# narendasan/irl-maxent

Hardware: AMD Instinct MI355X
Metric: IRL gradient steps/sec (VI + SVF sweep), NxN grid batch B (higher is better)
Workload: dtype f64

## Files before the change

irl-maxent_amd/csrc/cluster.h:

```cpp
#pragma once

#include <hip/hip_runtime.h>
#include <stdint.h>

#include "common.h"

namespace irlmx {

constexpr int kCT = 1024;
constexpr int kSptMax = 6;
constexpr int kPairThreads = 512;
constexpr int kSptMaxPair = 12;
constexpr int kSptMaxQuadFwd = 12;
constexpr int kSptMaxQuadBwd = 16;
constexpr int kSptMaxQuadBwdCW = 20;
constexpr int kTMax = 16;
constexpr int kSoloBwdT = 256;
constexpr int kRescaleEvery = 32;
constexpr size_t kMaxLdsBytes = 160 * 1024;
constexpr int kSumSlots = kRescaleEvery < 8 ? 8 : kRescaleEvery + 1;
static_assert(kSumSlots > kRescaleEvery, "summary slots must outlast the rescale period");
constexpr int kSumRows = kSumSlots + 2;
constexpr int kXccRow = kSumSlots, kFullRow = kSumSlots + 1;
constexpr size_t kClusterStaticLds = 128;
constexpr int kModeFwd = 0;
constexpr int kModeBwd = 1;

struct ClusterArgs {
  int W, H, S, A;
  int R, G, C, T;
  int b0;
  int nb;
  int btot;
  int emax;
  int tab_shared;
  const double* wgt;
  const double* row_val;
  const double* vin;
  const uint8_t* term;
  const int32_t* bad;
  const unsigned long long* growth;
  double eps;
  long long max_iter;
  long long n_sweeps;
  int rescale;
  unsigned long long* gran;
  unsigned long long* sgran;
  int xcd_group;
  unsigned salt;
  int* err;
  int n_resident;
  unsigned long long gather_ticks;
  int test_drop;
  int eager_summary;
  unsigned long long* stamps;
  double* out;
  int64_t* iters;
  int32_t* status;
};

struct ClusterPlan {
  int R, G, C, T, per_launch, spt, emax;
  size_t lds;
  int pair;
  int nt;
};

typedef unsigned int u32x4 __attribute__((ext_vector_type(4)));
constexpr int kPollSleep = 1;
constexpr int kGatherPerThread = 4;

#ifndef IRLMX_GRAN_PAR_PAD
#define IRLMX_GRAN_PAR_PAD -1
#endif
#ifndef IRLMX_GRAN_INST_PAD
#define IRLMX_GRAN_INST_PAD -1
#endif
__host__ __device__ inline size_t gran_par_pad(int W) { return IRLMX_GRAN_PAR_PAD >= 0 ? IRLMX_GRAN_PAR_PAD : (W == 128 ? 24 : 0); }
__host__ __device__ inline size_t gran_inst_pad(int W) { return IRLMX_GRAN_INST_PAD >= 0 ? IRLMX_GRAN_INST_PAD : (W == 128 ? 40 : 0); }
__host__ __device__ inline size_t gran_par_len(int W, int H) { return (size_t)H * W + gran_par_pad(W); }
__host__ __device__ inline size_t gran_inst_len(int W, int H) { return 2 * gran_par_len(W, H) + gran_inst_pad(W); }

struct Gran {
  __amdgpu_buffer_rsrc_t r;
#if IRLMX_DEVICE_CHECKS
  unsigned bytes;
#endif
};
__device__ inline Gran gran_rsrc(const void* base, unsigned bytes) {
  Gran g;
  g.r = __builtin_amdgcn_make_buffer_rsrc(const_cast<void*>(base), 0, (int)bytes, 0x00020000);
#if IRLMX_DEVICE_CHECKS
  g.bytes = bytes;
#endif
  return g;
}
#if IRLMX_DEVICE_CHECKS
__device__ inline bool gran_in(const Gran& g, unsigned off) { return g.bytes >= 16u && off <= g.bytes - 16u; }
#endif
__device__ inline unsigned long long dbits(double v) { return (unsigned long long)__double_as_longlong(v); }
__device__ inline void gran_store(const Gran& g, unsigned off, unsigned long long v, unsigned tag, bool plain) {
  if (!IRLMX_DCHECK(gran_in(g, off), kCheckGranule)) return;
  const u32x4 x = {(unsigned)v, tag, (unsigned)(v >> 32), tag};
  if (plain) __builtin_amdgcn_raw_buffer_store_b128(x, g.r, (int)off, 0, 0);
  else __builtin_amdgcn_raw_buffer_store_b128(x, g.r, (int)off, 0, 16 );
}
constexpr unsigned long long kGatherTicks = 2000000000ull;
// ... 100 lines not shown
```

irl-maxent_amd/csrc/cluster.hip:

```cpp

#include <hip/hip_runtime.h>

#include <algorithm>
#include <atomic>
#include <cmath>
#include <cstdio>
#include <cstdlib>
#include <type_traits>

#include "cluster.h"
#include "common.h"

namespace irlmx {

template <int CTRL>
__device__ inline double dpp_shift_f64(double x) {
  const long long b = __double_as_longlong(x);
  const int lo = __builtin_amdgcn_update_dpp(0, (int)(b & 0xffffffffLL), CTRL, 0xF, 0xF, true);
  const int hi = __builtin_amdgcn_update_dpp(0, (int)(b >> 32), CTRL, 0xF, 0xF, true);
  return __longlong_as_double(((long long)hi << 32) | (long long)(unsigned)lo);
}

template <int MODE, int SPT, int WT, int LAY, int NT>
__global__ void __launch_bounds__(NT) cluster_kernel(ClusterArgs a) {
  constexpr bool PAIR = LAY >= 1, COLS = LAY >= 2;
  constexpr bool CW = LAY == 4;
  constexpr int CPL = LAY >= 3 ? 4 : 2;
  static_assert(LAY != 1 || (SPT % 2 == 0 && (WT == 64 || WT == 128)), "pair rows: even SPT, width 64/128");
  static_assert(LAY != 2 || (SPT % 2 == 0 && (WT == 64 || WT == 128)), "column pairs: even SPT, width 64/128");
  static_assert(LAY != 3 || (SPT % 4 == 0 && (WT == 128 || WT == 256)), "column quads: SPT % 4, width 128/256");
  static_assert(LAY != 4 || (MODE == kModeBwd && SPT % 4 == 0 && WT == 256), "compact weights: backward, width 256");
  constexpr int RW = COLS ? SPT / CPL : 1;
  constexpr int HW = COLS ? WT / CPL : 1;
  constexpr int NB = COLS ? NT / HW : 1;
  constexpr int QW = CPL / 2;
  constexpr bool kProof = MODE == kModeFwd && COLS;
  constexpr int kProofRow = RW / 2;
  constexpr bool kLdsSides = COLS && CPL == 2 && MODE == kModeFwd;
  extern __shared__ __attribute__((aligned(16))) unsigned char smem[];
  const int W = WT ? WT : a.W;
  const int H = a.H, S = a.S;
  int lin = blockIdx.x;
  if (a.xcd_group) {
    const int g = blockIdx.x % 8, k = blockIdx.x / 8;
    const int il = g + 8 * (k / a.C);
    if (il >= a.nb) return;
    lin = il * a.C + k % a.C;
  }
  const int tile = lin % a.C;
  const int inst = a.b0 + lin / a.C;
  const int tid = threadIdx.x;
  {
    __shared__ int resident;
    if (tid == 0) resident = coresident(a.err + 1, a.n_resident) ? 1 : 0;
    __syncthreads();
    if (!resident) {
      if (tid == 0) atomicOr(a.err, kErrNotResident);
      return;
    }
  }
  if (lin == a.test_drop) return;
  const int r0 = tile * a.R, r1 = min(H, r0 + a.R);
  const int e0 = max(0, r0 - a.G), e1 = min(H, r1 + a.G);
  const int E = (e1 - e0) * W;
  if (!IRLMX_DCHECK(0 <= e0 && e0 <= r0 && r0 < r1 && r1 <= e1 && e1 <= H && E <= a.emax && E <= SPT * NT,
                    kCheckTile))
    return;
  const int own0 = (r0 - e0) * W, own1 = (r1 - e0) * W;
  const int pubA1 = min(own1, own0 + a.G * W), pubB0 = max(pubA1, own1 - a.G * W);
  const int base = e0 * W;
  const int pad = PAIR ? W : W + 1;
  const int blen = a.emax + 2 * pad;
  const int cp = COLS ? tid % HW : 0, bb = COLS ? tid / HW : 0;
  auto slot_state = [&](int j) {
    if (COLS) return (bb * RW + j / CPL) * W + CPL * cp + j % CPL;
    return PAIR ? 2 * (tid + (j >> 1) * NT) + (j & 1) : tid + j * NT;
  };
  double* bufA = (double*)smem;
  double* bufB = bufA + (COLS ? 0 : blen);
  double* snap = bufB + blen;
  constexpr int kBndLen = COLS ? 2 * (NB + 2) * 2 * HW * QW : 0;
  double2* bnd = CW ? (double2*)bufA : (double2*)(snap + (MODE == kModeFwd ? a.emax : 0));
  unsigned char* tail = CW ? (unsigned char*)bufA + max((size_t)blen * sizeof(double), (size_t)kBndLen * sizeof(double2))
                           : (unsigned char*)(bnd + kBndLen);
  double2* wmid = (double2*)tail;
  double2* zrow = wmid + (CW ? NB * RW * HW : 0);
  unsigned long long* red = (unsigned long long*)(zrow + (CW ? HW * QW : 0));
  int* lflag = (int*)(red + 3);

  const size_t iS = (size_t)inst * S;
  if (MODE == kModeFwd && a.bad[inst]) {
    for (int l = own0 + tid; l < own1; l += NT) a.out[iS + base + l] = __longlong_as_double(0x7ff8000000000000LL);
    if (tile == 0 && tid == 0) { a.iters[inst] = 1; a.status[inst] = IRLMX_NONFINITE; }
    return;
  }

  double w[CW ? 1 : SPT][kStencilK];
  double wc[CW ? SPT : 1][3];
  double edge_w[CW ? 2 * RW : 1];
  double c0[MODE == kModeFwd ? SPT : 1];
  const size_t wbase = iS * kStencilK;
#pragma unroll
  for (int j = 0; j < SPT; ++j) {
    const int l = slot_state(j);
    if (MODE == kModeFwd) c0[MODE == kModeFwd ? j : 0] = 0.0;
    if constexpr (CW) {
#pragma unroll
      for (int k = 0; k < 3; ++k) wc[j][k] = 0.0;
      if (l < E) {
        const int s = base + l;
        const int x = s % W;
        wc[j][0] = a.wgt[wbase + (size_t)(x + 1 < W ? 1 : 2) * S + s];
        wc[j][1] = a.wgt[wbase + (size_t)3 * S + s];
        wc[j][2] = a.wgt[wbase + (size_t)4 * S + s];
      }
#pragma unroll
      for (int k = 0; k < 3; ++k) asm volatile("" : "+v"(wc[j][k]));
    } else {
#pragma unroll
      for (int k = 0; k < kStencilK; ++k) w[j][k] = 0.0;
      if (l < E) {
        const int s = base + l;
        if (MODE == kModeFwd) c0[MODE == kModeFwd ? j : 0] = a.vin[iS + s];
#pragma unroll
        for (int k = 0; k < kStencilK; ++k) w[j][k] = a.wgt[wbase + (size_t)k * S + s];
      }
#pragma unroll
      for (int k = 0; k < kStencilK; ++k) asm volatile("" : "+v"(w[j][k]));
      if (MODE == kModeFwd) asm volatile("" : "+v"(c0[MODE == kModeFwd ? j : 0]));
    }
  }
  if constexpr (CW) {
#pragma unroll
    for (int r = 0; r < RW; ++r) {
      edge_w[2 * r] = 0.0;
      edge_w[2 * r + 1] = 0.0;
      const int l0 = slot_state(r * CPL), l3 = slot_state(r * CPL + CPL - 1);
      const int y = e0 + l0 / W;
      const bool brow = l0 < E && (y == 0 || y == H - 1);
      if ((cp == 0 || brow) && l0 < E) edge_w[2 * r] = a.wgt[wbase + base + l0];
      if ((cp == HW - 1 || brow) && l3 < E) edge_w[2 * r + 1] = a.wgt[wbase + base + l3];
      asm volatile("" : "+v"(edge_w[2 * r]));
      asm volatile("" : "+v"(edge_w[2 * r + 1]));
    }
  }
  auto finish = [&](int j, double acc) { return MODE == kModeFwd ? c0[MODE == kModeFwd ? j : 0] + acc : acc; };
  bool wave_p0 = true;
  if constexpr (MODE == kModeFwd) {
    bool mine = false;
#pragma unroll
    for (int j = 0; j < SPT; ++j) mine |= !(c0[MODE == kModeFwd ? j : 0] == 0.0);
    wave_p0 = __builtin_amdgcn_readfirstlane(__builtin_amdgcn_ballot_w64(mine) != 0ull ? 1 : 0) != 0;
  }
  for (int i = tid; i < (COLS ? 1 : 2) * blen; i += NT) bufA[i] = 0.0;
  for (int i = tid; i < kBndLen; i += NT) bnd[i] = make_double2(0.0, 0.0);
  if constexpr (CW) {
    static_assert(!CW || CPL == 4, "compact weights: column quads");
    for (int i = tid; i < HW * QW; i += NT) zrow[i] = make_double2(0.0, 0.0);
#pragma unroll
    for (int r = 0; r < RW; ++r) {
      const int l1 = slot_state(r * CPL + 1);
      const int y = e0 + l1 / W;
      const bool brow = l1 < E && (y == 0 || y == H - 1);
      wmid[(bb * RW + r) * HW + cp] = brow ? make_double2(a.wgt[wbase + base + l1], a.wgt[wbase + base + l1 + 1])
                                           : make_double2(0.0, 0.0);
    }
  }
  __syncthreads();
  for (int l = tid; l < E; l += NT) {
    double v0 = 0.0;
    if (MODE == kModeBwd) v0 = a.term[iS + base + l] ? 1.0 : 0.0;
    bufA[pad + l] = v0;
    bufB[pad + l] = v0;
    if (MODE == kModeFwd) snap[l] = v0;
  }
  if (tid < 3) red[tid] = 0ull;
  if (tid == 0) lflag[0] = 0;
  double cv[PAIR ? SPT : 1];
#pragma unroll
  for (int j = 0; j < (PAIR ? SPT : 1); ++j) {
    const int l = slot_state(j);
    cv[j] = (PAIR && MODE == kModeBwd && l < E) ? (a.term[iS + base + l] ? 1.0 : 0.0) : 0.0;
  }
  auto reload = [&](const double* buf) {
    if (PAIR) {
#pragma unroll
      for (int j = 0; j < (PAIR ? SPT : 1); ++j) cv[j] = buf[pad + slot_state(j)];
    }
  };

  unsigned own_bits = 0, pub_bits = 0, ext_bits = 0;
#pragma unroll
  for (int j = 0; j < SPT; ++j) {
    const int l = slot_state(j);
    const bool own = l >= own0 && l < own1;
    own_bits |= (own ? 1u : 0u) << j;
    ext_bits |= (l < E ? 1u : 0u) << j;
    pub_bits |= (((l >= own0 && l < pubA1) || (l >= pubB0 && l < own1)) ? 1u : 0u) << j;
  }

  constexpr bool kUniformSlots = LAY == 1 ? WT == 128 : (COLS && HW == 64);
  auto slot_bits = [&](unsigned b) {
    if constexpr (kUniformSlots) {
      b = (unsigned)__builtin_amdgcn_readfirstlane((int)b);
      asm volatile("" : "+s"(b));
    } else {
      asm volatile("" : "+v"(b));
    }
    return b;
  };

  int T = a.T;
  int p_max = 1;
  if (MODE == kModeBwd) {
    const double g = bits_double(a.growth[inst]);
    const double d = bits_double(a.growth[a.btot + inst]);
    if (a.rescale && isfinite(g)) {
      int cap = 1 << 20;
      if (g > 1.0) cap = max(1, (int)floor(900.0 / log2(g)) - 1);
      if (d > 0.0 && d < 1.0) cap = min(cap, max(1, (int)floor(900.0 / -log2(d)) - 1));
      if (d < 0.0) cap = min(cap, kTMax);
      T = max(1, min(T, cap));
      p_max = d < 0.0 ? 1 : max(1, min(kRescaleEvery, cap / T));
    }
  }
  __syncthreads();

  const double eps = a.eps;
  auto sweep = [&](const double* __restrict__ din, double* __restrict__ dout, int i, unsigned& flags) {
    const unsigned ob = slot_bits(own_bits);
    double dmax = 0.0;
    auto account = [&](int j, double nv, double self) {
      if (MODE == kModeFwd && ((ob >> j) & 1u)) dmax = fmax(dmax, fabs(nv - self));
    };
    if constexpr (PAIR && !COLS) {
#pragma unroll
      for (int jp = 0; jp < SPT / 2; ++jp) {
        const int l = 2 * (tid + jp * NT);
        const double2 up = *reinterpret_cast<const double2*>(din + l);
        const double2 dn = *reinterpret_cast<const double2*>(din + 2 * W + l);
        const double va = cv[2 * jp], vb = cv[2 * jp + 1];
        const double lft = dpp_shift_f64<0x138>(vb);
        const double rgt = dpp_shift_f64<0x130>(va);
        const double* wa = w[CW ? 0 : 2 * jp];
        const double* wb = w[CW ? 0 : 2 * jp + 1];
        double acc = fma(wa[0], va, 0.0);
        acc = fma(wa[1], vb, acc);
        acc = fma(wa[2], lft, acc);
        acc = fma(wa[3], dn.x, acc);
        acc = fma(wa[4], up.x, acc);
        const double na = finish(2 * jp, acc);
        acc = fma(wb[0], vb, 0.0);
        acc = fma(wb[1], rgt, acc);
        acc = fma(wb[2], va, acc);
        acc = fma(wb[3], dn.y, acc);
        acc = fma(wb[4], up.y, acc);
        const double nb = finish(2 * jp + 1, acc);
        *reinterpret_cast<double2*>(dout + W + l) = make_double2(na, nb);
        account(2 * jp, na, va);
        account(2 * jp + 1, nb, vb);
        cv[2 * jp] = na;
        cv[2 * jp + 1] = nb;
      }
    } else {
#pragma unroll
      for (int j = 0; j < SPT; ++j) {
        const int l = tid + j * NT;
        const double* q = din + l + 1;
        const double self = q[W];
        double acc = fma(w[CW ? 0 : j][0], self, 0.0);
        acc = fma(w[CW ? 0 : j][1], q[W + 1], acc);
        acc = fma(w[CW ? 0 : j][2], q[W - 1], acc);
        acc = fma(w[CW ? 0 : j][3], q[2 * W], acc);
        acc = fma(w[CW ? 0 : j][4], q[0], acc);
        const double nv = finish(j, acc);
        dout[pad + l] = nv;
        account(j, nv, self);
      }
    }
    if (MODE == kModeFwd) flags |= ((dmax > eps) ? 1u : 0u) << i;
    __syncthreads();
  };

  double cw[COLS ? SPT : 1];
  auto bnd_at = [&](int par, int band, int e) { return bnd + ((((size_t)par * (NB + 2) + band) * 2 + e) * HW + cp) * QW; };
  auto cols_sweep = [&](const double (&src)[COLS ? SPT : 1], double (&dst)[COLS ? SPT : 1], int i,
                        unsigned& flags, auto p0tag, auto fulltag) {
    constexpr bool kP0 = decltype(p0tag)::value;
    constexpr bool kFull = decltype(fulltag)::value;
    if constexpr (COLS) {
      const unsigned ob = slot_bits(own_bits);
      double dmax = 0.0;
      double2 wm_pf[CW ? RW : 1];
      if constexpr (CW) {
#pragma unroll
        for (int r = 0; r < RW; ++r) wm_pf[r] = wmid[(bb * RW + r) * HW + cp];
      }
      auto account = [&](int j, double nv, double self) {
        if (!kFull && j / CPL != kProofRow) return;
        if constexpr (MODE == kModeFwd && kUniformSlots) {
          if ((ob >> j) & 1u) {
            asm volatile("");
            dmax = fmax(dmax, fabs(nv - self));
          }
        } else if (MODE == kModeFwd && ((ob >> j) & 1u)) {
          dmax = fmax(dmax, fabs(nv - self));
        }
      };
      {
        double2* t = bnd_at(i & 1, bb + 1, 0);
        double2* u = bnd_at(i & 1, bb + 1, 1);
#pragma unroll
        for (int q = 0; q < QW; ++q) {
          t[q] = make_double2(src[2 * q], src[2 * q + 1]);
          u[q] = make_double2(src[SPT - CPL + 2 * q], src[SPT - CPL + 2 * q + 1]);
        }
      }
      constexpr bool kBwdPairs12 = CPL == 2 && MODE == kModeBwd && SPT >= 12;
      constexpr bool kPinStores = CPL == 2 && MODE == kModeBwd && (SPT <= 8 || kBwdPairs12);
      if constexpr (kPinStores) __builtin_amdgcn_sched_barrier(0);
      if (MODE == kModeFwd && i == 0) {
        const unsigned xb = slot_bits(ext_bits);
#pragma unroll
        for (int jp = 0; jp < SPT / 2; ++jp)
          if ((xb >> (2 * jp)) & 1u)
            *reinterpret_cast<double2*>(snap + slot_state(2 * jp)) = make_double2(src[2 * jp], src[2 * jp + 1]);
      }
      double above[CPL], below[CPL];
      double side[2][2];
      constexpr bool kPin = CPL == 2 && !kBwdPairs12;
      auto edges_in = [&]() {
        if (kPin) __builtin_amdgcn_sched_barrier(0);
        __syncthreads();
        if (kPin) __builtin_amdgcn_sched_barrier(0);
        const double2* t = (CW && bb == 0) ? zrow + cp * QW : bnd_at(i & 1, bb, 1);
        const double2* u = (CW && bb == NB - 1) ? zrow + cp * QW : bnd_at(i & 1, bb + 2, 0);
#pragma unroll
        for (int q = 0; q < QW; ++q) {
          const double2 x = t[q];
// ... 26 lines not shown
          double acc[CPL];
          if constexpr (CW) {
            const double2 wm = wm_pf[jr];
            acc[0] = fma(edge_w[2 * jr], v[0], 0.0);
            acc[1] = fma(wm.x, v[1], 0.0);
            acc[2] = fma(wm.y, v[2], 0.0);
            acc[CPL - 1] = fma(edge_w[2 * jr + 1], v[CPL - 1], 0.0);
#pragma unroll
            for (int c = 0; c < CPL; ++c) acc[c] = fma(wc[jr * CPL + c][0], c + 1 < CPL ? v[c + 1 < CPL ? c + 1 : 0] : rgt, acc[c]);
#pragma unroll
            for (int c = 0; c < CPL; ++c) acc[c] = fma(wc[jr * CPL + c][0], c > 0 ? v[c > 0 ? c - 1 : 0] : lft, acc[c]);
#pragma unroll
            for (int c = 0; c < CPL; ++c) acc[c] = fma(wc[jr * CPL + c][1], dn[c], acc[c]);
#pragma unroll
            for (int c = 0; c < CPL; ++c) acc[c] = fma(wc[jr * CPL + c][2], up[c], acc[c]);
          } else {
#pragma unroll
            for (int c = 0; c < CPL; ++c) acc[c] = fma(w[CW ? 0 : jr * CPL + c][0], v[c], 0.0);
#pragma unroll
            for (int c = 0; c < CPL; ++c) acc[c] = fma(w[CW ? 0 : jr * CPL + c][1], c + 1 < CPL ? v[c + 1 < CPL ? c + 1 : 0] : rgt, acc[c]);
#pragma unroll
            for (int c = 0; c < CPL; ++c) acc[c] = fma(w[CW ? 0 : jr * CPL + c][2], c > 0 ? v[c > 0 ? c - 1 : 0] : lft, acc[c]);
#pragma unroll
            for (int c = 0; c < CPL; ++c) acc[c] = fma(w[CW ? 0 : jr * CPL + c][3], dn[c], acc[c]);
#pragma unroll
            for (int c = 0; c < CPL; ++c) acc[c] = fma(w[CW ? 0 : jr * CPL + c][4], up[c], acc[c]);
          }
#pragma unroll
          for (int c = 0; c < CPL; ++c) {
            dst[jr * CPL + c] = kP0 ? finish(jr * CPL + c, acc[c]) : acc[c];
            account(jr * CPL + c, dst[jr * CPL + c], v[c]);
          }
        }
      };
      constexpr int step = CPL == 2 ? 2 : 1;
      constexpr int n_int = RW >= 3 ? (RW - 2 + step - 1) / step : 0;
      constexpr int kPre = (CW || kBwdPairs12) ? n_int
                           : (CPL == 2 && MODE == kModeFwd && SPT <= 8) ? 0
                                                                       : (n_int + 1) / 2;
#pragma unroll
      for (int s = 0; s < n_int; ++s) {
        if (s == kPre) edges_in();
        const int jp = 1 + s * step;
        rows(jp, jp + step - 1 <= RW - 2 ? jp + step - 1 : jp);
      }
      if constexpr (kPre >= n_int) edges_in();
      if constexpr (RW >= 2) {
        if constexpr (CPL == 2) rows(RW - 1, 0);
        else { rows(RW - 1, RW - 1); rows(0, 0); }
      } else {
        rows(0, 0);
      }
      if (MODE == kModeFwd) flags |= ((dmax > eps) ? 1u : 0u) << i;
    }
  };

  const size_t gpl = gran_par_len(W, H);
  const Gran rg = gran_rsrc(a.gran + (size_t)inst * 2 * gran_inst_len(W, H), 32u * (unsigned)gpl);
  const unsigned rgw = (unsigned)W;
  const unsigned gbase = (unsigned)e0 * rgw;
  auto gidx = [&](int l) { return gbase + (unsigned)(l / W) * rgw + (unsigned)(l % W); };
  const Gran rs = gran_rsrc(a.sgran + (size_t)inst * 2 * kSumRows * a.H, 16u * kSumRows * (unsigned)a.H);
  const int ng0 = own0, ng = own0 + (E - own1);
  const unsigned salt = (a.salt & 0xFFFu) << 20;
  bool plain = false;
  {
    unsigned xcc;
    asm volatile("s_getreg_b32 %0, hwreg(HW_REG_XCC_ID)" : "=s"(xcc));
    xcc &= 0xFu;
    const unsigned htag = salt | 0xFFFFFu;
    if (tid == 0) gran_store(rs, ((unsigned)kXccRow * (unsigned)a.H + (unsigned)tile) * 16u, xcc, htag, false);
    bool ok = true;
    if (tid < kWave) {
      unsigned long long diff = 0ull;
      for (int t0 = 0; t0 < a.C; t0 += kWave) {
        unsigned long long v[1] = {xcc};
        unsigned off[1] = {((unsigned)kXccRow * (unsigned)a.H + (unsigned)(t0 + tid)) * 16u};
        ok &= gran_gather<1>(rs, rs, off, t0 + tid < a.C ? 1u : 0u, htag, v, a.gather_ticks);
        diff |= v[0] ^ xcc;
      }
      diff = wave_or_u64(diff);
      if (tid == 0) { red[2] = diff; lflag[1] = ok ? 0 : 1; }
    }
    __syncthreads();
    if (lflag[1]) { if (tid == 0) atomicOr(a.err, 1); return; }
    plain = a.xcd_group && red[2] == 0ull;
    __syncthreads();
  }

  double* cur = bufA;
  double* oth = bufB;
  long long done = 0;
  __shared__ unsigned long long st_acc[8], ts_l[1];
  const bool stamps = a.stamps != nullptr && tid == 0;
  if (stamps) {
    for (int k = 0; k < 8; ++k) st_acc[k] = 0ull;
    ts_l[0] = stamp_now();
  }
  unsigned long long& ts = ts_l[0];
  auto stamp = [&](int k) {
    if (stamps) { const unsigned long long t = stamp_now(); st_acc[k] += t - ts; ts = t; }
  };
  auto stamp_flush = [&]() {
    if (stamps) {
      for (int k = 0; k < 5; ++k) a.stamps[(size_t)lin * 8 + k] = st_acc[k];
      a.stamps[(size_t)lin * 8 + 5] = plain ? 1 : 0;
// ... 3 lines not shown
  };
  const long long total = MODE == kModeBwd ? a.n_sweeps : -1;
  int rescale_in = 1;
  auto run_sweeps = [&](int n, unsigned& fl) {
    if constexpr (COLS) {
      int i = 0;
      for (; i + 1 < n; i += 2) {
        cols_sweep(cv, cw, i, fl, std::true_type{}, std::true_type{});
        cols_sweep(cw, cv, i + 1, fl, std::true_type{}, std::true_type{});
      }
      if (i < n) {
        cols_sweep(cv, cw, i, fl, std::true_type{}, std::true_type{});
#pragma unroll
        for (int j = 0; j < (COLS ? SPT : 1); ++j) cv[j] = cw[j];
      }
    } else {
      for (int i = 0; i < n; ++i) {
        sweep(cur, oth, i, fl);
        double* t = cur; cur = oth; oth = t;
      }
    }
  };
  auto restore = [&]() {
    for (int l = tid; l < E; l += NT) cur[pad + l] = snap[l];
    __syncthreads();
    reload(cur);
  };
  auto block_sweeps = [&](unsigned& fl, const int n, auto fulltag) {
    if constexpr (COLS && MODE == kModeFwd) {
      auto go = [&](auto p0tag) {
        int i = 0;
        for (; i + 1 < n; i += 2) {
          cols_sweep(cv, cw, i, fl, p0tag, fulltag);
          cols_sweep(cw, cv, i + 1, fl, p0tag, fulltag);
        }
        if (i < n) {
          cols_sweep(cv, cw, i, fl, p0tag, fulltag);
#pragma unroll
          for (int j = 0; j < (COLS ? SPT : 1); ++j) cv[j] = cw[j];
        }
      };
      if (MODE == kModeFwd && ((decltype(fulltag)::value && kProof) || wave_p0)) go(std::true_type{});
      else go(std::false_type{});
    }
  };
  for (int m = 0;; ++m) {
    int Tm = T;
    if (MODE == kModeBwd) Tm = (int)min<long long>((long long)T, total - done);
    unsigned flags = 0;
    const bool resc = MODE == kModeBwd && a.rescale && (rescale_in <= 1 || done + Tm >= total);
    double mxd = 0.0;
    if constexpr (COLS) {
      if constexpr (MODE == kModeBwd) {
        int i = 0;
        for (; i + 1 < Tm; i += 2) {
          cols_sweep(cv, cw, i, flags, std::false_type{}, std::true_type{});
          cols_sweep(cw, cv, i + 1, flags, std::false_type{}, std::true_type{});
        }
        if (i < Tm) {
          cols_sweep(cv, cw, i, flags, std::false_type{}, std::true_type{});
#pragma unroll
          for (int j = 0; j < (COLS ? SPT : 1); ++j) cv[j] = cw[j];
        }
      } else {
        block_sweeps(flags, Tm, std::integral_constant<bool, !kProof>{});
      }
      if constexpr (CW) __syncthreads();
    } else {
      run_sweeps(Tm, flags);
    }
    if (MODE == kModeFwd) {
      const unsigned ob = slot_bits(own_bits);
      bool nf = false;
#pragma unroll
      for (int j = 0; j < SPT; ++j)
        if ((ob >> j) & 1u) nf |= !isfinite(PAIR ? cv[PAIR ? j : 0] : cur[pad + slot_state(j)]);
      if (nf) flags |= 1u << 31;
    }
    if (resc) {
      const unsigned ob = slot_bits(own_bits);
#pragma unroll
      for (int j = 0; j < SPT; ++j)
        if ((ob >> j) & 1u) mxd = fmax(mxd, fabs(PAIR ? cv[PAIR ? j : 0] : cur[pad + slot_state(j)]));
    }
    stamp(0);
    if (stamps) st_acc[4] += 1;
    const unsigned tag = salt | (((unsigned)m + 1u) & 0xFFFFFu);
    const unsigned gpar = (unsigned)(m & 1) * (unsigned)gpl;
    const bool solo = WT == 64 && a.C == 1;
    auto store_rows = [&]() {
      for (int l = own0 + tid; l < pubA1; l += NT)
        gran_store(rg, (gpar + gidx(l)) * 16u, dbits(cur[pad + l]), tag, plain);
      for (int l = pubB0 + tid; l < own1; l += NT)
        gran_store(rg, (gpar + gidx(l)) * 16u, dbits(cur[pad + l]), tag, plain);
    };
    if constexpr (COLS) {
      const unsigned pb = slot_bits(pub_bits);
#pragma unroll
      for (int jp = 0; jp < SPT / 2; ++jp)
        if ((pb >> (2 * jp)) & 1u)
          *reinterpret_cast<double2*>(cur + pad + slot_state(2 * jp)) =
              make_double2(cv[PAIR ? 2 * jp : 0], cv[PAIR ? 2 * jp + 1 : 0]);
    } else if constexpr (PAIR) {
      const unsigned pb = slot_bits(pub_bits);
#pragma unroll
      for (int j = 0; j < SPT; ++j)
        if ((pb >> j) & 1u)
          gran_store(rg, (gpar + gidx(slot_state(j))) * 16u, dbits(cv[PAIR ? j : 0]), tag, plain);
    } else {
      store_rows();
    }
    if (stamps) { const unsigned long long t = stamp_now(); st_acc[5] += t - ts; }
    unsigned* red32 = (unsigned*)red;
    if (tid == 0) red32[2 + ((m + 1) & 1)] = 0u;
    if (MODE == kModeFwd) {
      const unsigned wf = wave_reduce_u32<1>(flags) & (((1u << Tm) - 1) | (1u << 31));
      if ((tid & (kWave - 1)) == 0 && wf) atomicOr(&red32[m & 1], wf);
    } else if (resc) {
      const unsigned wc = wave_reduce_u32<0>(scale_code(mxd));
      if ((tid & (kWave - 1)) == 0 && wc) atomicMax(&red32[m & 1], wc);
    }
    if (stamps) { const unsigned long long t = stamp_now(); st_acc[6] += t - ts; }
    __syncthreads();
    if (!solo) {
      if (tid == 0) gran_store(rs, ((unsigned)(m % kSumSlots) * (unsigned)a.H + (unsigned)tile) * 16u, red32[m & 1], tag, plain);
      if constexpr (COLS && CPL == 2) {
        store_rows();
      } else if constexpr (COLS) {
        constexpr int kPub = 4;
        const int nA = pubA1 - own0, ntot = nA + (own1 - pubB0);
        for (int k0 = 0; k0 < ntot; k0 += kPub * NT) {
          int ls[kPub];
          double vv[kPub];
#pragma unroll
          for (int i = 0; i < kPub; ++i) {
            const int k = k0 + tid + i * NT;
            ls[i] = k < nA ? own0 + k : (k < ntot ? pubB0 + (k - nA) : -1);
            vv[i] = cur[pad + (ls[i] >= 0 ? ls[i] : 0)];
          }
#pragma unroll
          for (int i = 0; i < kPub; ++i)
            if (ls[i] >= 0) gran_store(rg, (gpar + gidx(ls[i])) * 16u, dbits(vv[i]), tag, plain);
        }
      }
    }
    stamp(1);
    bool ok = true;
    constexpr int GPT = PAIR ? kGatherPerThread : 1;
    const bool need_summary = a.eager_summary || MODE == kModeFwd || resc;
    auto gather = [&]() {
      for (int k0 = 0; k0 < max(ng, 1); k0 += GPT * NT) {
        unsigned off[GPT + 1];
// ... 53 lines not shown
          if (!solo) {
            if (tid == 0)
              gran_store(rs, ((unsigned)kFullRow * (unsigned)a.H + (unsigned)tile) * 16u, (unsigned)lflag[2], tag,
                         plain);
            if (tid < a.C) {
              unsigned long long v[1];
              const unsigned off[1] = {((unsigned)kFullRow * (unsigned)a.H + (unsigned)tid) * 16u};
              ok2 = gran_gather<1>(rs, rs, off, 1u, tag, v, a.gather_ticks);
              if (ok2) atomicOr(reinterpret_cast<unsigned*>(&lflag[3]), (unsigned)v[0]);
            }
          } else if (tid == 0) {
            lflag[3] = lflag[2];
          }
          if (!ok2) { lflag[0] = 1; atomicOr(a.err, 1); }
          __syncthreads();
          if (lflag[0]) return;
          msk = (unsigned)__builtin_amdgcn_readfirstlane(lflag[3]);
        }
      }
      if ((msk & live) != live || (a.max_iter > 0 && done + Tm >= a.max_iter)) {
        for (int i = 0; i < Tm; ++i) {
          const bool cap = a.max_iter > 0 && done + i + 1 >= a.max_iter;
          if (!((msk >> i) & 1u) || cap) { conv = i + 1; break; }
        }
      }
      if (conv) {
        restore();
        unsigned scratch = 0;
        run_sweeps(conv, scratch);
        if (COLS) {
          const unsigned ob = slot_bits(own_bits);
#pragma unroll
          for (int j = 0; j < SPT; ++j)
            if ((ob >> j) & 1u) a.out[iS + base + slot_state(j)] = cv[PAIR ? j : 0];
        } else {
          for (int l = own0 + tid; l < own1; l += NT) a.out[iS + base + l] = cur[pad + l];
        }
        stamp(3);
        stamp_flush();
        if (tile == 0 && tid == 0) {
          const bool big = (msk >> (conv - 1)) & 1u;
          a.iters[inst] = done + conv;
          a.status[inst] = big ? IRLMX_MAXITER : IRLMX_OK;
        }
        return;
      }
    }
    done += Tm;
    const int e_scale = resc ? code_exponent(summary) : 0;
    if (MODE == kModeBwd) rescale_in = resc ? ((e_scale <= 0 && m >= 3) ? p_max : 1) : rescale_in - 1;
    if constexpr (PAIR) {
      const unsigned ob = slot_bits(own_bits), xb = slot_bits(ext_bits);
#pragma unroll
      for (int jp = 0; jp < SPT / 2; ++jp) {
        const int l = slot_state(2 * jp);
        const bool own = (ob >> (2 * jp)) & 1u, ext = (xb >> (2 * jp)) & 1u;
        double2 v = make_double2(cv[PAIR ? 2 * jp : 0], cv[PAIR ? 2 * jp + 1 : 0]);
        if (!own && ext) v = *reinterpret_cast<const double2*>(cur + pad + l);
        if (MODE == kModeBwd && e_scale) {
          v.x = ldexp(v.x, e_scale);
          v.y = ldexp(v.y, e_scale);
          if (ext && !COLS) *reinterpret_cast<double2*>(cur + pad + l) = v;
        }
        if (MODE == kModeFwd && ext && !COLS) *reinterpret_cast<double2*>(snap + l) = v;
        cv[PAIR ? 2 * jp : 0] = v.x;
        cv[PAIR ? 2 * jp + 1 : 0] = v.y;
      }
    } else if (MODE == kModeFwd || e_scale) {
      for (int l = tid; l < E; l += NT) {
        double v = cur[pad + l];
        if (MODE == kModeBwd) cur[pad + l] = v = ldexp(v, e_scale);
        if (MODE == kModeFwd) snap[l] = v;
      }
    }
    if constexpr (!COLS || CW || MODE == kModeBwd) __syncthreads();
    stamp(3);
    if (MODE == kModeBwd && done >= total) break;
  }
  stamp_flush();

  if (MODE == kModeBwd) {
    if (COLS) {
      const unsigned xb = slot_bits(ext_bits);
#pragma unroll
      for (int jp = 0; jp < SPT / 2; ++jp)
        if ((xb >> (2 * jp)) & 1u)
          *reinterpret_cast<double2*>(cur + pad + slot_state(2 * jp)) = make_double2(cv[PAIR ? 2 * jp : 0], cv[PAIR ? 2 * jp + 1 : 0]);
      if constexpr (CW) {
        for (int l = tid; l < pad; l += NT) cur[l] = 0.0;
        for (int l = pad + E + tid; l < blen; l += NT) cur[l] = 0.0;
      }
      __syncthreads();
    }
    const int A = a.A;
    const size_t tb = a.tab_shared ? 0 : (size_t)inst;
    for (int l = own0 + tid; l < own1; l += NT) {
      const int s = base + l;
      const double* q = cur + l + (pad - W);
      const double er = exp(a.vin[iS + s]);
      double za[8];
      double zsum = 0.0;
      for (int act = 0; act < A; ++act) {
        const double* rv = a.row_val + ((tb * A + act) * kStencilK) * (size_t)S + s;
        double acc = fma(rv[0], q[W], 0.0);
        acc = fma(rv[(size_t)1 * S], q[W + 1], acc);
        acc = fma(rv[(size_t)2 * S], q[W - 1], acc);
        acc = fma(rv[(size_t)3 * S], q[2 * W], acc);
        acc = fma(rv[(size_t)4 * S], q[0], acc);
        za[act] = er * acc;
        zsum += za[act];
      }
      for (int act = 0; act < A; ++act) a.out[(iS + s) * A + act] = za[act] / zsum;
    }
    if (tile == 0 && tid == 0) a.status[inst] = IRLMX_OK;
  }
}

}

namespace irlmx {

constexpr unsigned long long kNoDecayBound = 0xBFF0000000000000ull;
__global__ void bwd_growth_kernel(const double* __restrict__ bw, int W, int S, int B,
                                  unsigned long long* __restrict__ growth) {
  const int b = blockIdx.x;
  const double* wb = bw + (size_t)b * kStencilK * S;
  unsigned long long mx = 0ull, mn = ~0ull;
  unsigned dead = 0u;
  for (int s = threadIdx.x; s < S; s += blockDim.x) {
    double row = 0.0;
    for (int k = 0; k < kStencilK; ++k) {
      const double x = wb[(size_t)k * S + s];
      row += x;
      if (x > 0.0) mn = min(mn, abs_bits(x));
    }
    mx = max(mx, abs_bits(row));
    const int x = s % W;
    const bool feeds = wb[s] > 0.0 || (x > 0 && wb[(size_t)1 * S + s - 1] > 0.0) ||
// ... 167 lines not shown
        case 16: return (void*)&cluster_kernel<MODE, 16, 256, 4, kPairThreads>;
        case 20: return (void*)&cluster_kernel<MODE, 20, 256, 4, kPairThreads>;
      }
    }
    return nullptr;
  }
  if (layout == 3) {
    if (W == 128) return cluster_fn_quad<MODE, 128>(spt);
    if (W == 256) return cluster_fn_quad<MODE, 256>(spt);
    return nullptr;
  }
  if (layout == 1 || layout == 2) {
    if (W == 64) return layout == 1 ? cluster_fn_pair<MODE, 64, 1>(spt) : cluster_fn_pair<MODE, 64, 2>(spt);
    if (W == 128) return layout == 1 ? cluster_fn_pair<MODE, 128, 1>(spt) : cluster_fn_pair<MODE, 128, 2>(spt);
    return nullptr;
  }
  switch (W) {
    case 64: return cluster_fn_w<MODE, 64>(spt);
    case 128: return cluster_fn_w<MODE, 128>(spt);
    case 256: return cluster_fn_w<MODE, 256>(spt);
  }
  return cluster_fn_w<MODE, 0>(spt);
}

int cluster_run(int mode, const ClusterPlan& plan, ClusterArgs a, int B, hipStream_t st) {
  ClusterPlan p = plan;
  void* fn;
  fn = mode == kModeFwd ? cluster_fn<kModeFwd>(p.spt, a.W, p.pair, p.nt) : cluster_fn<kModeBwd>(p.spt, a.W, p.pair, p.nt);
  const int nt = p.nt;
  if (!fn) { set_error("cluster: no kernel for spt=%d", p.spt); return IRLMX_EINVAL; }
  hipError_t e = hipFuncSetAttribute(fn, hipFuncAttributeMaxDynamicSharedMemorySize, (int)p.lds);
  if (e != hipSuccess) return hip_fail(e, "cluster hipFuncSetAttribute");
  int per_cu = 0;
  e = hipOccupancyMaxActiveBlocksPerMultiprocessor(&per_cu, (const void*)fn, nt, p.lds);
  if (e != hipSuccess) return hip_fail(e, "cluster occupancy");
  const int resident = per_cu * device_cus();
  if (p.C * p.per_launch > resident) {
    set_error("cluster: %d workgroups cannot be co-resident (%d)", p.C * p.per_launch, resident);
    return IRLMX_EINVAL;
  }
  a.R = p.R; a.G = p.G; a.C = p.C; a.T = p.T; a.emax = p.emax; a.btot = B;
  unsigned long long* stamps = nullptr;
  const int nwg = p.C * std::min(p.per_launch, B);
  if (env_int("IRLMX_STAMPS", 0)) {
    e = hipMallocAsync((void**)&stamps, sizeof(unsigned long long) * 8 * nwg, st);
    if (e != hipSuccess) return hip_fail(e, "stamps alloc");
    (void)hipMemsetAsync(stamps, 0, sizeof(unsigned long long) * 8 * nwg, st);
  }
  a.stamps = stamps;
  const LaunchTestKnobs tk = launch_test_knobs();
  a.test_drop = tk.drop;
  a.gather_ticks = tk.gather_ticks;
  a.eager_summary = env_int("IRLMX_EAGER_SUMMARY", 0) ? 1 : 0;
  for (int b0 = 0; b0 < B; b0 += p.per_launch) {
    const int nb = std::min(p.per_launch, B - b0);
    a.b0 = b0;
    a.nb = nb;
    a.n_resident = nb * p.C + tk.extra_resident;
    if (b0 > 0) {
      e = hipMemsetAsync(a.err + 1, 0, 2 * sizeof(int), st);
      if (e != hipSuccess) return hip_fail(e, "cluster rendezvous reset");
    }
    a.xcd_group = xcd_groupable(nb, p.C) && env_int("IRLMX_XCD_GROUP", 1) != 0;
    a.salt = g_salt.fetch_add(1, std::memory_order_relaxed);
    void* args[] = {&a};
    const int grid = a.xcd_group ? 8 * ((nb + 7) / 8) * p.C : nb * p.C;
    e = hipLaunchKernel(fn, dim3(grid), dim3(nt), args, p.lds, st);
    if (e != hipSuccess) return hip_fail(e, "cluster launch");
    count_event(IRLMX_CTR_CLUSTER_LAUNCHES);
  }
  int err = 0;
  e = hipMemcpyAsync(&err, a.err, sizeof(int), hipMemcpyDeviceToHost, st);
  if (e == hipSuccess) e = hipStreamSynchronize(st);
  if (e != hipSuccess) return hip_fail(e, "cluster sync");
  if (stamps) {
    unsigned long long* h = (unsigned long long*)malloc(sizeof(unsigned long long) * 8 * nwg);
    (void)hipMemcpy(h, stamps, sizeof(unsigned long long) * 8 * nwg, hipMemcpyDeviceToHost);
    double acc[8] = {0, 0, 0, 0, 0, 0, 0, 0};
    for (int g = 0; g < nwg; ++g)
      for (int k = 0; k < 8; ++k) acc[k] += (double)h[(size_t)g * 8 + k] / nwg;
    fprintf(stderr, "[irlmx stamps] %s%s mode=%d R=%d G=%d C=%d spt=%d blocks=%.0f  cycles/block: sweeps %.0f  publish %.0f  "
                    "wait %.0f  refresh %.0f  same-xcd %.2f  (publish: stores %.0f, summary %.0f)\n", "lds", p.pair == 4 ? "-quads-cw" : p.pair == 3 ? "-quads" : (p.pair == 2 ? "-cols" : (p.pair == 1 ? "-pair" : "")), mode, p.R, p.G, p.C, p.spt,
            acc[4], acc[0] / acc[4], acc[1] / acc[4], acc[2] / acc[4], acc[3] / acc[4], acc[5], acc[6] / acc[4],
            (acc[7] - acc[6]) / acc[4]);
    if (p.C <= 8) {
      for (int t = 0; t < p.C; ++t) {
        double ta[5] = {0, 0, 0, 0, 0};
        int n = 0;
        for (int g = t; g < nwg; g += p.C, ++n)
          for (int k = 0; k < 5; ++k) ta[k] += (double)h[(size_t)g * 8 + k];
        if (n && ta[4] > 0)
          fprintf(stderr, "[irlmx stamps]   tile %d: sweeps %.0f  publish %.0f  wait %.0f  refresh %.0f\n", t,
                  ta[0] / ta[4], ta[1] / ta[4], ta[2] / ta[4], ta[3] / ta[4]);
      }
    }
    free(h);
    (void)hipFree(stamps);
  }
  if (err & kErrNotResident) {
    count_event(IRLMX_CTR_RERUN_NOT_RESIDENT);
    return kClusterNotResident;
  }
  if (err & 1) {
    if (env_int("IRLMX_STRICT_EXCHANGE", 0)) {
      set_error("cluster: halo exchange timed out (workgroups not co-resident?)");
      return IRLMX_EHIP;
// ... 10 lines not shown
```

Measured before the change: 2744.

## Add trapezoidal halo-shrinking sweep schedule for backward W=128 column kernel

For the backward column-layout kernel at W=128 with R=32, T=G=8, each wave is assigned a band of rows that differs by tile position. Per sweep it computes only the rows that still influence the owned rows, because halo rows stop mattering as sweeps progress (a trapezoid in time). Compile-time tables with static_asserts check that the liveness pattern and the per-SIMD load balance are correct. This cuts redundant halo arithmetic but adds a switch over band kinds, more register slots (NS=14), and code-size growth from many template instantiations.

```diff
diff --git a/irl-maxent_amd/csrc/cluster.h b/irl-maxent_amd/csrc/cluster.h
--- a/irl-maxent_amd/csrc/cluster.h
+++ b/irl-maxent_amd/csrc/cluster.h
@@ -53,6 +53,7 @@
   unsigned long long gather_ticks;
   int test_drop;
   int eager_summary;
+  int trap_noskip;
   unsigned long long* stamps;
   double* out;
   int64_t* iters;
diff --git a/irl-maxent_amd/csrc/cluster.hip b/irl-maxent_amd/csrc/cluster.hip
--- a/irl-maxent_amd/csrc/cluster.hip
+++ b/irl-maxent_amd/csrc/cluster.hip
@@ -20,6 +20,74 @@
   const int hi = __builtin_amdgcn_update_dpp(0, (int)(b >> 32), CTRL, 0xF, 0xF, true);
   return __longlong_as_double(((long long)hi << 32) | (long long)(unsigned)lo);
 }
+
+constexpr int kTrapT = 8, kTrapR = 32, kTrapRowsMax = 7;
+constexpr int trap_h(int k) { return (k == 0 || k == 3 || k == 7) ? 7 : (k == 5) ? 5 : k == 6 ? 4 : 6; }
+constexpr int trap_d0(int k) { return k == 0 ? 8 : k == 1 ? 1 : k == 2 ? -4 : k == 3 ? 2 : 0; }
+constexpr int trap_ds(int k) { return (k == 0 || k == 1) ? -1 : (k == 2 || k == 3) ? 1 : 0; }
+constexpr int trap_dist(int k, int j) { return trap_d0(k) + trap_ds(k) * j < 0 ? 0 : trap_d0(k) + trap_ds(k) * j; }
+constexpr bool trap_live(int k, int j, int I) { return I == 0 || trap_dist(k, j) <= kTrapT - I; }
+constexpr int trap_kind(int tk, int b) {
+  if (tk == 0) return b == 6 ? 2 : b == 7 ? 3 : b % 2 == 0 ? 5 : 6;
+  if (tk == 1) return b == 0 ? 0 : b == 1 ? 1 : b == 6 ? 2 : b == 7 ? 3 : (b == 2 || b == 5) ? 4 : 5;
+  return b == 0 ? 0 : b == 1 ? 1 : b % 2 == 0 ? 5 : 6;
+}
+constexpr int trap_first(int tk, int b) {
+  int f = 0;
+  for (int q = 0; q < b; ++q) f += trap_h(trap_kind(tk, q));
+  return f;
+}
+constexpr int trap_band_of_wave(int w) {
+  return w == 0 ? 0 : w == 4 ? 1 : w == 1 ? 7 : w == 5 ? 6 : w == 2 ? 2 : w == 6 ? 3 : w == 3 ? 4 : 5;
+}
+constexpr int trap_tile_rows(int tk) { return tk == 1 ? 48 : 40; }
+constexpr int trap_own0(int tk) { return tk == 0 ? 0 : 8; }
+constexpr bool trap_needed(int tk, int row, int I) {
+  for (int r = trap_own0(tk); r < trap_own0(tk) + kTrapR; ++r)
+    if ((r > row ? r - row : row - r) <= kTrapT - I) return true;
+  return false;
+}
+constexpr bool trap_table_ok() {
+  for (int tk = 0; tk < 3; ++tk) {
+    int seen = 0;
+    for (int w = 0; w < 8; ++w) seen |= 1 << trap_band_of_wave(w);
+    if (seen != 0xFF) return false;
+    if (trap_first(tk, 8) != trap_tile_rows(tk)) return false;
+    for (int b = 0; b < 8; ++b) {
+      const int k = trap_kind(tk, b), f = trap_first(tk, b);
+      if (trap_h(k) > kTrapRowsMax || trap_h(k) < 3) return false;
+      for (int I = 1; I <= kTrapT; ++I)
+        for (int j = -1; j <= trap_h(k); ++j) {
+          const int row = f + j;
+          if (row < 0 || row >= trap_tile_rows(tk)) continue;
+          if (trap_live(k, j, I) != trap_needed(tk, row, I)) return false;
+        }
+    }
+  }
+  return true;
+}
+constexpr int trap_simd_rows(int tk, int I) {
+  int mx = 0;
+  for (int s = 0; s < 4; ++s) {
+    int n = 0;
+    for (int w = s; w < 8; w += 4) {
+      const int k = trap_kind(tk, trap_band_of_wave(w));
+      for (int j = 0; j < trap_h(k); ++j) n += trap_live(k, j, I) ? 1 : 0;
+    }
+    mx = n > mx ? n : mx;
+  }
+  return mx;
+}
+constexpr bool trap_simd_ok() {
+  constexpr int want[kTrapT] = {12, 11, 11, 11, 11, 11, 11, 11};
+  for (int I = 1; I <= kTrapT; ++I) {
+    if (trap_simd_rows(1, I) != want[I - 1]) return false;
+    if (trap_simd_rows(0, I) > want[I - 1] || trap_simd_rows(2, I) > want[I - 1]) return false;
+  }
+  return true;
+}
+static_assert(trap_table_ok(), "trapezoid bands: a row is computed at sweep I exactly when an owned row depends on it");
+static_assert(trap_simd_ok(), "trapezoid bands: busiest SIMD carries 12, 11, 11, 11, 11, 11, 11, 11 rows");
 
 template <int MODE, int SPT, int WT, int LAY, int NT>
 __global__ void __launch_bounds__(NT) cluster_kernel(ClusterArgs a) {
@@ -36,6 +104,8 @@
   constexpr int QW = CPL / 2;
   constexpr bool kProof = MODE == kModeFwd && COLS;
   constexpr int kProofRow = RW / 2;
+  constexpr bool kTrap = MODE == kModeBwd && LAY == 2 && WT == 128 && SPT == 12 && NT == 512;
+  constexpr int NS = kTrap ? 2 * kTrapRowsMax : SPT;
   constexpr bool kLdsSides = COLS && CPL == 2 && MODE == kModeFwd;
   extern __shared__ __attribute__((aligned(16))) unsigned char smem[];
   const int W = WT ? WT : a.W;
@@ -72,7 +142,23 @@
   const int pad = PAIR ? W : W + 1;
   const int blen = a.emax + 2 * pad;
   const int cp = COLS ? tid % HW : 0, bb = COLS ? tid / HW : 0;
+  const bool trap = kTrap && a.R == kTrapR && a.G == kTrapT && a.T == kTrapT && a.C >= 2 && H == a.C * kTrapR;
+  int tband = 0, tfirst = 0, tkind = 0, trows = 0;
+  if constexpr (kTrap) {
+    const int tk = tile == 0 ? 0 : tile == a.C - 1 ? 2 : 1;
+    tband = __builtin_amdgcn_readfirstlane(trap_band_of_wave(bb));
+    tfirst = __builtin_amdgcn_readfirstlane(trap_first(tk, tband));
+    tkind = __builtin_amdgcn_readfirstlane(trap_kind(tk, tband));
+    trows = __builtin_amdgcn_readfirstlane(trap_h(tkind));
+  }
+  auto slot_ok = [&](int j) {
+    if constexpr (kTrap) return trap ? j / CPL < trows : j < SPT;
+    return true;
+  };
   auto slot_state = [&](int j) {
+    if constexpr (kTrap) {
+      if (trap) return (tfirst + j / CPL) * W + CPL * cp + j % CPL;
+    }
     if (COLS) return (bb * RW + j / CPL) * W + CPL * cp + j % CPL;
     return PAIR ? 2 * (tid + (j >> 1) * NT) + (j & 1) : tid + j * NT;
   };
@@ -95,13 +181,13 @@
     return;
   }
 
-  double w[CW ? 1 : SPT][kStencilK];
+  double w[CW ? 1 : NS][kStencilK];
   double wc[CW ? SPT : 1][3];
   double edge_w[CW ? 2 * RW : 1];
   double c0[MODE == kModeFwd ? SPT : 1];
   const size_t wbase = iS * kStencilK;
 #pragma unroll
-  for (int j = 0; j < SPT; ++j) {
+  for (int j = 0; j < NS; ++j) {
     const int l = slot_state(j);
     if (MODE == kModeFwd) c0[MODE == kModeFwd ? j : 0] = 0.0;
     if constexpr (CW) {
@@ -119,7 +205,7 @@
     } else {
 #pragma unroll
       for (int k = 0; k < kStencilK; ++k) w[j][k] = 0.0;
-      if (l < E) {
+      if (slot_ok(j) && l < E) {
         const int s = base + l;
         if (MODE == kModeFwd) c0[MODE == kModeFwd ? j : 0] = a.vin[iS + s];
 #pragma unroll
@@ -176,27 +262,27 @@
   }
   if (tid < 3) red[tid] = 0ull;
   if (tid == 0) lflag[0] = 0;
-  double cv[PAIR ? SPT : 1];
-#pragma unroll
-  for (int j = 0; j < (PAIR ? SPT : 1); ++j) {
+  double cv[PAIR ? NS : 1];
+#pragma unroll
+  for (int j = 0; j < (PAIR ? NS : 1); ++j) {
     const int l = slot_state(j);
-    cv[j] = (PAIR && MODE == kModeBwd && l < E) ? (a.term[iS + base + l] ? 1.0 : 0.0) : 0.0;
+    cv[j] = (PAIR && MODE == kModeBwd && slot_ok(j) && l < E) ? (a.term[iS + base + l] ? 1.0 : 0.0) : 0.0;
   }
   auto reload = [&](const double* buf) {
     if (PAIR) {
 #pragma unroll
-      for (int j = 0; j < (PAIR ? SPT : 1); ++j) cv[j] = buf[pad + slot_state(j)];
+      for (int j = 0; j < (PAIR ? NS : 1); ++j) cv[j] = buf[pad + slot_state(j)];
     }
   };
 
   unsigned own_bits = 0, pub_bits = 0, ext_bits = 0;
 #pragma unroll
-  for (int j = 0; j < SPT; ++j) {
+  for (int j = 0; j < NS; ++j) {
     const int l = slot_state(j);
-    const bool own = l >= own0 && l < own1;
+    const bool ok = slot_ok(j), own = ok && l >= own0 && l < own1;
     own_bits |= (own ? 1u : 0u) << j;
-    ext_bits |= (l < E ? 1u : 0u) << j;
-    pub_bits |= (((l >= own0 && l < pubA1) || (l >= pubB0 && l < own1)) ? 1u : 0u) << j;
+    ext_bits |= (ok && l < E ? 1u : 0u) << j;
+    pub_bits |= ((ok && ((l >= own0 && l < pubA1) || (l >= pubB0 && l < own1))) ? 1u : 0u) << j;
   }
 
   constexpr bool kUniformSlots = LAY == 1 ? WT == 128 : (COLS && HW == 64);
@@ -282,9 +368,9 @@
     __syncthreads();
   };
 
-  double cw[COLS ? SPT : 1];
+  double cw[COLS ? NS : 1];
   auto bnd_at = [&](int par, int band, int e) { return bnd + ((((size_t)par * (NB + 2) + band) * 2 + e) * HW + cp) * QW; };
-  auto cols_sweep = [&](const double (&src)[COLS ? SPT : 1], double (&dst)[COLS ? SPT : 1], int i,
+  auto cols_sweep = [&](const double (&src)[COLS ? NS : 1], double (&dst)[COLS ? NS : 1], int i,
                         unsigned& flags, auto p0tag, auto fulltag) {
     constexpr bool kP0 = decltype(p0tag)::value;
     constexpr bool kFull = decltype(fulltag)::value;
@@ -417,6 +503,87 @@
         rows(0, 0);
       }
       if (MODE == kModeFwd) flags |= ((dmax > eps) ? 1u : 0u) << i;
+    }
+  };
+
+  auto trap_sweep = [&](const double (&src)[COLS ? NS : 1], double (&dst)[COLS ? NS : 1], auto ktag, auto itag,
+                        const int par) {
+    if constexpr (kTrap) {
+      constexpr int K = decltype(ktag)::value, I = decltype(itag)::value, HB = trap_h(K);
+      constexpr bool top_live = trap_live(K, 0, I), bot_live = trap_live(K, HB - 1, I);
+      if constexpr (trap_live(K, -1, I)) *bnd_at(par, tband + 1, 0) = make_double2(src[0], src[1]);
+      if constexpr (trap_live(K, HB, I)) *bnd_at(par, tband + 1, 1) = make_double2(src[2 * HB - 2], src[2 * HB - 1]);
+      __builtin_amdgcn_sched_barrier(0);
+      double above[2] = {0.0, 0.0}, below[2] = {0.0, 0.0};
+      auto rows = [&](int j1, int j2) {
+#pragma unroll
+        for (int h = 0; h < 2; ++h) {
+          if (h == 1 && j2 == j1) break;
+          const int jr = h == 0 ? j1 : j2;
+          const double* v = src + jr * 2;
+          const double* up = jr == 0 ? above : src + (jr > 0 ? jr - 1 : 0) * 2;
+          const double* dn = jr == HB - 1 ? below : src + (jr + 1 < HB ? jr + 1 : HB - 1) * 2;
+          const double lft = dpp_shift_f64<0x138>(v[1]);
+          const double rgt = dpp_shift_f64<0x130>(v[0]);
+          double acc[2];
+#pragma unroll
+          for (int c = 0; c < 2; ++c) acc[c] = fma(w[CW ? 0 : jr * 2 + c][0], v[c], 0.0);
+          acc[0] = fma(w[CW ? 0 : jr * 2][1], v[1], acc[0]);
+          acc[1] = fma(w[CW ? 0 : jr * 2 + 1][1], rgt, acc[1]);
+          acc[0] = fma(w[CW ? 0 : jr * 2][2], lft, acc[0]);
+          acc[1] = fma(w[CW ? 0 : jr * 2 + 1][2], v[0], acc[1]);
+#pragma unroll
+          for (int c = 0; c < 2; ++c) acc[c] = fma(w[CW ? 0 : jr * 2 + c][3], dn[c], acc[c]);
+#pragma unroll
+          for (int c = 0; c < 2; ++c) acc[c] = fma(w[CW ? 0 : jr * 2 + c][4], up[c], acc[c]);
+          dst[jr * 2] = acc[0];
+          dst[jr * 2 + 1] = acc[1];
+        }
+      };
+      constexpr int lo = [] { int j = 1; while (j <= HB - 2 && !trap_live(K, j, I)) ++j; return j; }();
+      constexpr int hi = [] { int j = HB - 2; while (j >= 1 && !trap_live(K, j, I)) --j; return j; }();
+#pragma unroll
+      for (int j = lo; j <= hi; j += 2) rows(j, j + 1 <= hi ? j + 1 : j);
+      __syncthreads();
+      if constexpr (top_live) {
+        const double2 x = *bnd_at(par, tband, 1);
+        above[0] = x.x; above[1] = x.y;
+      }
+      if constexpr (bot_live) {
+        const double2 y = *bnd_at(par, tband + 2, 0);
+        below[0] = y.x; below[1] = y.y;
+      }
+      if constexpr (top_live && bot_live) rows(HB - 1, 0);
+      else if constexpr (bot_live) rows(HB - 1, HB - 1);
+      else if constexpr (top_live) rows(0, 0);
+    }
+  };
+  auto trap_block = [&](auto ktag, auto nktag, const int Tm) {
+    if constexpr (kTrap) {
+      using std::integral_constant;
+      if (Tm == kTrapT && !a.trap_noskip) {
+        trap_sweep(cv, cw, ktag, integral_constant<int, 1>{}, 0);
+        trap_sweep(cw, cv, ktag, integral_constant<int, 2>{}, 1);
+        trap_sweep(cv, cw, ktag, integral_constant<int, 3>{}, 0);
+        trap_sweep(cw, cv, ktag, integral_constant<int, 4>{}, 1);
+        trap_sweep(cv, cw, ktag, integral_constant<int, 5>{}, 0);
+        trap_sweep(cw, cv, ktag, integral_constant<int, 6>{}, 1);
+        trap_sweep(cv, cw, ktag, integral_constant<int, 7>{}, 0);
+        trap_sweep(cw, cv, ktag, integral_constant<int, 8>{}, 1);
+      } else {
+        constexpr int HB = trap_h(decltype(nktag)::value);
+        const std::integral_constant<int, 0> all{};
+        int i = 0;
+        for (; i + 1 < Tm; i += 2) {
+          trap_sweep(cv, cw, nktag, all, 0);
+          trap_sweep(cw, cv, nktag, all, 1);
+        }
+        if (i < Tm) {
+          trap_sweep(cv, cw, nktag, all, 0);
+#pragma unroll
+          for (int j = 0; j < 2 * HB; ++j) cv[j] = cw[j];
+        }
+      }
     }
   };
 
@@ -526,15 +693,28 @@
     double mxd = 0.0;
     if constexpr (COLS) {
       if constexpr (MODE == kModeBwd) {
-        int i = 0;
-        for (; i + 1 < Tm; i += 2) {
-          cols_sweep(cv, cw, i, flags, std::false_type{}, std::true_type{});
-          cols_sweep(cw, cv, i + 1, flags, std::false_type{}, std::true_type{});
-        }
-        if (i < Tm) {
-          cols_sweep(cv, cw, i, flags, std::false_type{}, std::true_type{});
-#pragma unroll
-          for (int j = 0; j < (COLS ? SPT : 1); ++j) cv[j] = cw[j];
+        if (kTrap && trap) {
+          using std::integral_constant;
+          switch (tkind) {
+            case 0: trap_block(integral_constant<int, 0>{}, integral_constant<int, 7>{}, Tm); break;
+            case 1: trap_block(integral_constant<int, 1>{}, integral_constant<int, 4>{}, Tm); break;
+            case 2: trap_block(integral_constant<int, 2>{}, integral_constant<int, 4>{}, Tm); break;
+            case 3: trap_block(integral_constant<int, 3>{}, integral_constant<int, 7>{}, Tm); break;
+            case 4: trap_block(integral_constant<int, 4>{}, integral_constant<int, 4>{}, Tm); break;
+            case 5: trap_block(integral_constant<int, 5>{}, integral_constant<int, 5>{}, Tm); break;
+            default: trap_block(integral_constant<int, 6>{}, integral_constant<int, 6>{}, Tm); break;
+          }
+        } else {
+          int i = 0;
+          for (; i + 1 < Tm; i += 2) {
+            cols_sweep(cv, cw, i, flags, std::false_type{}, std::true_type{});
+            cols_sweep(cw, cv, i + 1, flags, std::false_type{}, std::true_type{});
+          }
+          if (i < Tm) {
+            cols_sweep(cv, cw, i, flags, std::false_type{}, std::true_type{});
+#pragma unroll
+            for (int j = 0; j < (COLS ? SPT : 1); ++j) cv[j] = cw[j];
+          }
         }
       } else {
         block_sweeps(flags, Tm, std::integral_constant<bool, !kProof>{});
@@ -554,7 +734,7 @@
     if (resc) {
       const unsigned ob = slot_bits(own_bits);
 #pragma unroll
-      for (int j = 0; j < SPT; ++j)
+      for (int j = 0; j < NS; ++j)
         if ((ob >> j) & 1u) mxd = fmax(mxd, fabs(PAIR ? cv[PAIR ? j : 0] : cur[pad + slot_state(j)]));
     }
     stamp(0);
@@ -571,7 +751,7 @@
     if constexpr (COLS) {
       const unsigned pb = slot_bits(pub_bits);
 #pragma unroll
-      for (int jp = 0; jp < SPT / 2; ++jp)
+      for (int jp = 0; jp < NS / 2; ++jp)
         if ((pb >> (2 * jp)) & 1u)
           *reinterpret_cast<double2*>(cur + pad + slot_state(2 * jp)) =
               make_double2(cv[PAIR ? 2 * jp : 0], cv[PAIR ? 2 * jp + 1 : 0]);
@@ -731,7 +911,7 @@
     if constexpr (PAIR) {
       const unsigned ob = slot_bits(own_bits), xb = slot_bits(ext_bits);
 #pragma unroll
-      for (int jp = 0; jp < SPT / 2; ++jp) {
+      for (int jp = 0; jp < NS / 2; ++jp) {
         const int l = slot_state(2 * jp);
         const bool own = (ob >> (2 * jp)) & 1u, ext = (xb >> (2 * jp)) & 1u;
         double2 v = make_double2(cv[PAIR ? 2 * jp : 0], cv[PAIR ? 2 * jp + 1 : 0]);
@@ -762,7 +942,7 @@
     if (COLS) {
       const unsigned xb = slot_bits(ext_bits);
 #pragma unroll
-      for (int jp = 0; jp < SPT / 2; ++jp)
+      for (int jp = 0; jp < NS / 2; ++jp)
         if ((xb >> (2 * jp)) & 1u)
           *reinterpret_cast<double2*>(cur + pad + slot_state(2 * jp)) = make_double2(cv[PAIR ? 2 * jp : 0], cv[PAIR ? 2 * jp + 1 : 0]);
       if constexpr (CW) {
@@ -1036,6 +1216,7 @@
   a.test_drop = tk.drop;
   a.gather_ticks = tk.gather_ticks;
   a.eager_summary = env_int("IRLMX_EAGER_SUMMARY", 0) ? 1 : 0;
+  a.trap_noskip = env_int("IRLMX_TRAP_NOSKIP", 0) ? 1 : 0;
   for (int b0 = 0; b0 < B; b0 += p.per_launch) {
     const int nb = std::min(p.per_launch, B - b0);
     a.b0 = b0;
```

New measurement: 2784, median of 6. +1.4%, better.
